# pcodec/pcodec

Measured on AMD Instinct MI355X. Metric: encode+decode GB/s (uncompressed) per chunk, u64/f64 2^18-elem, higher is better.
Workload: dtype u64

## Files before the change

### pcodec_amd/csrc/decode_fast.hip

```cpp
#include "decode_kernel.hip"
#include "pco_cursor.h"
#include "pco_index.h"

namespace pcogfx {

constexpr uint32_t kGrpWinOff = 0;
constexpr uint32_t kGrpVarOff = 448;
constexpr uint32_t kGrpTblOff = 640;
template <uint32_t KQ> struct WalkCfg {
  static constexpr uint32_t kGrpBytes = KQ == 8 ? 4912u : 9904u;
  static constexpr uint32_t kGrpTblBytes = kGrpBytes - kGrpTblOff;
  static constexpr uint32_t kWalkTmpOff = KQ * kGrpBytes;
  static constexpr uint32_t kWalkTmpObOff = kWalkTmpOff + 1056;
  static constexpr uint32_t kWalkLdsBytes = kWalkTmpObOff + 256;
  static constexpr uint32_t kRetryStatus = KQ == 8 ? 101u : 100u;
  static_assert(kGrpBytes % 16 == 0, "chunk slices must stay 16-byte aligned");
  static_assert(kWalkLdsBytes < 65536, "walk entries hold 16-bit LDS addresses");
};
template <uint32_t KQ> __device__ __forceinline__ uint8_t PCO_LDS* walk_lds() { return lds_base() + uni((uint32_t)(threadIdx.x >> 6)) * WalkCfg<KQ>::kWalkLdsBytes; }
__device__ __forceinline__ uint32_t walk_block_id() { return blockIdx.x * (blockDim.x >> 6) + uni((uint32_t)(threadIdx.x >> 6)); }
constexpr uint32_t kTrailDead = 0xffffffffu;
constexpr uint32_t kTrailDoneWord = 8;
constexpr uint32_t kTrailProgressStride = 32;
constexpr bool kTrailDefer = true;
constexpr uint32_t kTrailMaxBins = 64;
constexpr uint32_t kFastMaxBins = 256;
constexpr uint32_t kStatusRetryLegacy = 100;
constexpr uint32_t kStatusRetryK4 = 101;
constexpr uint32_t kStatusNeedHist = 102;
constexpr uint32_t kStatusEmptyRange = 103;

struct DecPlan {
  uint32_t status, n;
  uint32_t mode_kind, mode_k;
  uint64_t mode_base;
  uint32_t num_kind, dtype;
  uint32_t present[3], n_bins[3], max_ob[3], delta_kind[3], delta_order[3], nlps[3];
  uint32_t window_n_log, state_n_log;
  uint64_t moments[2][8];
  uint64_t consumed;
  uint32_t fused, more;
};
struct ReadRef { const uint64_t* from; uint64_t* to; };
struct ReadRec {
  uint32_t route;
  uint32_t b0;
  uint32_t resumed, pad;
  uint64_t mom[2][8];
  uint64_t end_row, end_bit;
  uint32_t end_states[3][4];
};
struct ResumeArgs { const ReadRef* refs; ReadRec* recs; uint32_t walk_cap; };
struct IndexRef { uint64_t* cursors; uint32_t every_batches, k; };
struct IndexArgs { const IndexRef* refs; };
constexpr uint64_t kBinsAreaPerVar = kFastMaxBins * 8 + kFastMaxBins;
constexpr uint64_t kBinsAreaPerTask = 3 * kBinsAreaPerVar;

__device__ __forceinline__ uint32_t make_wentry(uint32_t next_base, uint32_t sym, uint32_t btr, uint32_t ob) { return btr | (ob << 6) | (sym << 13) | (next_base << 21); }

template <class LV, uint32_t KQ>
__device__ __forceinline__ bool fast_build_var_impl(uint32_t q, uint32_t vi, MetaReader& mr, uint8_t PCO_GLOBAL* bins_out, uint32_t& status) {
  constexpr uint32_t kGrpBytes = WalkCfg<KQ>::kGrpBytes, kWalkTmpOff = WalkCfg<KQ>::kWalkTmpOff;
  const uint32_t lane = lane_id();
  uint8_t PCO_LDS* grp = walk_lds<KQ>() + q * kGrpBytes;
  VarInfo PCO_LDS* vinfo = (VarInfo PCO_LDS*)(grp + kGrpVarOff) + vi;
  const uint32_t asl = uni(vinfo->ans_size_log), n_bins = uni(vinfo->n_bins), latent_bits = uni(vinfo->latent_bits);
  const uint32_t T = 1u << asl;
  const uint32_t tbl_addr = (uint32_t)(uintptr_t)walk_lds<KQ>() + q * kGrpBytes + kGrpTblOff + uni(vinfo->off_nodes);
  uint32_t PCO_LDS* entries = (uint32_t PCO_LDS*)(grp + kGrpTblOff + uni(vinfo->off_nodes));
  uint8_t PCO_LDS* obs = walk_lds<KQ>() + WalkCfg<KQ>::kWalkTmpObOff;
  uint8_t PCO_LDS* ob0 = grp + kGrpTblOff + uni(vinfo->off_ob);
  uint32_t PCO_LDS* cum = (uint32_t PCO_LDS*)(walk_lds<KQ>() + kWalkTmpOff);
  uint64_t PCO_GLOBAL* g_low = (uint64_t PCO_GLOBAL*)(bins_out + (uint64_t)vi * kBinsAreaPerVar);
  uint8_t PCO_GLOBAL* g_ob = bins_out + (uint64_t)vi * kBinsAreaPerVar + kFastMaxBins * 8;
  const uint32_t obb = offset_bits_bits(latent_bits);
  const uint32_t bin_bits = asl + latent_bits + obb;
  const uint64_t bins_start = mr.bit;
  uint32_t bad = 0, max_ob = 0, carry = 0;
  for (uint32_t b0 = 0; b0 < n_bins; b0 += 64) {
    const uint32_t b = b0 + lane;
    uint32_t w = 0;
    if (b < n_bins) {
      const uint64_t at = bins_start + (uint64_t)b * bin_bits;
      w = (uint32_t)mr.peek(at, asl) + 1;
      const uint64_t lower = mr.peek(at + asl, latent_bits);
      const uint32_t ob = (uint32_t)mr.peek(at + asl + latent_bits, obb);
      if (ob > latent_bits) bad = 1;
      g_low[b] = lower; g_ob[b] = (uint8_t)ob; obs[b] = (uint8_t)ob;
      if (b == 0) ob0[0] = (uint8_t)ob;
      max_ob = max_ob > ob ? max_ob : ob;
    }
    const uint32_t incl = wave_incl_scan(w);
    if (b < n_bins) cum[b] = carry + incl - w;
    carry += wave_last(incl);
  }
  if (lane == 0) cum[n_bins] = carry;
  mr.bit = bins_start + (uint64_t)n_bins * bin_bits;
  max_ob = uni(wave_max_u32(max_ob));
  if (lane == 0) vinfo->max_ob = max_ob;
  if (!mr.in_bounds()) { status = PCO_GFX_INSUFFICIENT_DATA; return false; }
  if (uni(wave_or_u32(bad))) { status = PCO_GFX_CORRUPTION; return false; }
  if (n_bins == 0) { if (lane == 0) entries[0] = make_wentry(0, 0, 0, 0); wave_sync_lds(); return true; }
  if (carry != T) { status = PCO_GFX_CORRUPTION; return false; }
  wave_sync_lds();
  uint32_t stride = (3 * T) / 5; if ((stride & 1) == 0) stride += 1;
  for (uint32_t t = lane; t < T; t += 64) {
    uint32_t lo = 0, hi = n_bins;
    while (hi - lo > 1) { const uint32_t mid = (lo + hi) >> 1; if (cum[mid] <= t) lo = mid; else hi = mid; }
    entries[(stride * t) & (T - 1)] = lo;
  }
  wave_sync_lds();
// ... 195 lines not shown
  }
  if (!mr.drain_empty_byte()) { if (mr.in_bounds()) { fail(PCO_GFX_CORRUPTION); return; } }
  if (!mr.in_bounds()) { fail(PCO_GFX_INSUFFICIENT_DATA); return; }
  const uint32_t n_in_body = n > nlps[1] ? n - nlps[1] : 0;
  if (n_in_body > 0) for (int vi = 0; vi < 3; vi++) if (present[vi] && uni(vinfo[vi].n_bins) == 0) { fail(PCO_GFX_CORRUPTION); return; }
  out.mode_kind = mode_kind;
  if (lane == 0) {
    plan->status = PCO_GFX_OK; plan->n = n; plan->mode_kind = mode_kind; plan->mode_k = mode_k; plan->mode_base = (uint64_t)mode_base;
    plan->num_kind = num_kind; plan->dtype = dtype; plan->window_n_log = wlog; plan->state_n_log = slog; plan->consumed = 0; plan->fused = 0; plan->more = 0;
    for (int vi = 0; vi < 3; vi++) {
      plan->present[vi] = present[vi]; plan->n_bins[vi] = vinfo[vi].n_bins; plan->max_ob[vi] = vinfo[vi].max_ob;
      plan->delta_kind[vi] = vinfo[vi].delta_kind; plan->delta_order[vi] = vinfo[vi].delta_order; plan->nlps[vi] = nlps[vi];
    }
  }
  out.n = n; out.bitpos = mr.bit;
}

template <class L, uint32_t KQ>
__device__ __noinline__ void fast_front(const PcoGfxDecodeTask& task, uint32_t q, DecPlan PCO_GLOBAL* plan, uint8_t PCO_GLOBAL* bins_out, FrontOut& out, gcptr_u8 meta_p, uint64_t meta_len) { fast_front_impl<L, KQ, false>(task, q, plan, bins_out, out, meta_p, meta_len); }
template <class L, uint32_t KQ>
__device__ __noinline__ void fast_front_range(const PcoGfxDecodeTask& task, uint32_t q, DecPlan PCO_GLOBAL* plan, uint8_t PCO_GLOBAL* bins_out, FrontOut& out, gcptr_u8 meta_p, uint64_t meta_len) { fast_front_impl<L, KQ, false, true>(task, q, plan, bins_out, out, meta_p, meta_len); }

struct ResumeIn { uint64_t row, bitpos; uint32_t states[3][4]; uint32_t resumed; };
template <uint32_t KQ>
__device__ __noinline__ uint32_t resume_front(const uint64_t* from, uint32_t q, uint64_t page_n, uint32_t dtype, uint64_t page_len, uint64_t first, uint64_t count,
                                              uint64_t body_first_bit, uint32_t walk_cap, ReadRec* rec_g, ResumeIn& in) {
  const uint32_t lane = lane_id();
  ReadRec PCO_GLOBAL* rec = (ReadRec PCO_GLOBAL*)rec_g;
  const VarInfo PCO_LDS* vinfo = (const VarInfo PCO_LDS*)(walk_lds<KQ>() + q * WalkCfg<KQ>::kGrpBytes + kGrpVarOff);
  in.row = 0; in.bitpos = body_first_bit;
  uint32_t status = PCO_GFX_OK, resumed = 0;
  if (from != nullptr) {
    const uint64_t PCO_GLOBAL* cw = (const uint64_t PCO_GLOBAL*)from;
    uint64_t w[kCursorMomentWord];
#pragma unroll
    for (uint32_t i = 0; i < kCursorMomentWord; i++) w[i] = uni(cw[i]);
    uint32_t asl[3];
#pragma unroll
    for (int v = 0; v < 3; v++) asl[v] = uni(vinfo[v].present) ? uni(vinfo[v].ans_size_log) : 0u;
    status = cursor_verdict(w, kCursorFull, page_n, dtype, first, body_first_bit, page_len * 8, asl);
    if (status == PCO_GFX_OK) {
      resumed = 1; in.row = w[1]; in.bitpos = w[2];
#pragma unroll
      for (uint32_t v = 0; v < 3; v++) for (uint32_t j = 0; j < 4; j++) in.states[v][j] = cursor_state(w, v, j);
      if (lane < 16) rec->mom[lane >> 3][lane & 7] = cw[kCursorMomentWord + lane];
    }
  }
  if (status == PCO_GFX_OK && range_end_batch(first, count) - (in.row >> 8) > walk_cap) status = PCO_GFX_INVALID_ARGUMENT;
  in.resumed = status == PCO_GFX_OK ? resumed : 0u;
  if (lane == 0) { rec->route = status == PCO_GFX_OK ? 1u : 0u; rec->b0 = (uint32_t)(in.row >> 8); rec->resumed = resumed; rec->pad = 0; }
  return status;
}

struct WalkRegs {
  uint32_t saddr;
  uint32_t e;
  uint32_t bitaddr;
  uint32_t d0, d1, d2;
  uint32_t obsum, symacc;
};

__device__ __forceinline__ void walk_window(WalkRegs& r, uint32_t tot) {
  r.bitaddr += tot;
  const uint32_t PCO_LDS* w = (const uint32_t PCO_LDS*)(uintptr_t)((r.bitaddr >> 3) & ~3u);
  r.d0 = w[0]; r.d1 = w[1]; r.d2 = w[2];
}

template <bool kAgent>
__device__ __forceinline__ void store_syms(uint8_t PCO_GLOBAL* p, uint32_t __attribute__((ext_vector_type(4))) acc) {
  typedef uint32_t u32x4 __attribute__((ext_vector_type(4)));
  if constexpr (kAgent) {
    __asm__ volatile("global_store_dwordx4 %0, %1, off sc1" : : "v"(p), "v"(acc) : "memory");
  } else *(u32x4 PCO_GLOBAL*)p = acc;
}

struct QuadMasks { uint32_t m1, m2, m3, c63; };

template <int K, bool kTail>
__device__ __forceinline__ void walk_step(WalkRegs& r, const QuadMasks& m, uint32_t tbl_addr, bool chain_on) {
  uint32_t e = r.e;
  if (kTail) e = chain_on ? e : 0u;
  const uint32_t p = ((uint32_t)__builtin_amdgcn_update_dpp(0, (int)e, 0x111, 0xf, 0xf, true) & m.m1) +
                     ((uint32_t)__builtin_amdgcn_update_dpp(0, (int)e, 0x112, 0xf, 0xf, true) & m.m2) +
                     ((uint32_t)__builtin_amdgcn_update_dpp(0, (int)e, 0x113, 0xf, 0xf, true) & m.m3);
  const uint32_t x0 = __builtin_amdgcn_alignbit(r.d1, r.d0, r.bitaddr), x1 = __builtin_amdgcn_alignbit(r.d2, r.d1, r.bitaddr);
  const uint64_t xs = (((uint64_t)x1 << 32) | x0) >> (p & 63u);
  const uint32_t v = __builtin_amdgcn_ubfe((uint32_t)xs, 0u, e);
  const uint32_t next = tbl_addr + (((e >> 21) + v) << 2);
  if (kTail) r.saddr = chain_on ? next : r.saddr; else r.saddr = next;
  r.e = *(const uint32_t PCO_LDS*)(uintptr_t)r.saddr;
  __builtin_amdgcn_sched_barrier(0);
  const uint32_t t = p + e;
  walk_window(r, (uint32_t)__builtin_amdgcn_update_dpp(0, (int)t, 0xFF, 0xf, 0xf, true) & m.c63);
  if (K == 0) r.symacc = __builtin_amdgcn_ubfe(e, 13u, 8u); else r.symacc |= __builtin_amdgcn_ubfe(e, 13u, 8u) << (8 * K);
  r.obsum += __builtin_amdgcn_ubfe(e, 6u, 7u);
  __builtin_amdgcn_sched_barrier(0);
}

__device__ __forceinline__ uint32_t block_trail_kinds(const PcoGfxDecodeTask* tasks, const uint32_t* task_ids, uint32_t n_ids, uint32_t wb, const MetaRef* metas) {
  const uint32_t lane = lane_id(), bi = wb * 8 + (lane & 7u);
  bool one = false, two = false;
  if (lane < 8 && bi < n_ids) {
    const uint32_t ti = task_ids ? task_ids[bi] : bi;
    const PcoGfxDecodeTask t = tasks[ti];
    const bool wrapped = (t.flags & PCO_GFX_TASK_WRAPPED_PAGE) != 0;
    const uint32_t fmt = wrapped ? (t.flags >> 8) & 0xffu : ((t.flags & PCO_GFX_TASK_ONE_CHUNK) && ((t.flags >> 8) & 0xffu) ? (t.flags >> 8) & 0xffu : 4u);
    gcptr_u8 mp = (gcptr_u8)t.src + 4; uint64_t mlen = t.src_len >= 4 ? t.src_len - 4 : 0;
    if (wrapped) { if (metas != nullptr && metas[ti].p != nullptr) { mp = (gcptr_u8)metas[ti].p; mlen = metas[ti].len; } else { mp = (gcptr_u8)t.src; mlen = t.src_len; } }
    if ((t.flags & (PCO_GFX_TASK_META_ONLY | PCO_GFX_TASK_HAS_FILE_HEADER)) == 0 && mlen >= 20 && fmt >= 3 && fmt <= 4) {
      const uint64_t w = load_u64_le(mp);
      const uint32_t mode = (uint32_t)w & 15u;
      if (mode == kClassic) {
        const uint32_t dv = (uint32_t)(w >> 4) & 15u;
        const uint32_t n_bins = (uint32_t)(w >> (dv == kDeltaConsecutive ? 16 : 12)) & 0x7fffu;
        one = (dv == kDeltaNone || dv == kDeltaConsecutive) && n_bins > 1 && n_bins <= kTrailMaxBins;
      } else if (mode == kIntMult || mode == kFloatMult || mode == kFloatQuant) {
        const uint32_t at = 4u + (mode == kFloatQuant ? kBitsQuantK : (uint32_t)dtype_bits(t.dtype));
        const uint64_t w2 = load_u64_le(mp + (at >> 3));
        const uint32_t dv = (uint32_t)(w2 >> (at & 7u)) & 15u;
        two = dv == kDeltaNone || dv == kDeltaConsecutive;
      }
    }
  }
  return (uni((uint32_t)__any(one)) ? 1u : 0u) | (uni((uint32_t)__any(two)) ? 2u : 0u);
}
__device__ __forceinline__ bool block_has_trail_candidate(const PcoGfxDecodeTask* tasks, const uint32_t* task_ids, uint32_t n_ids, uint32_t wb, const MetaRef* metas) {
  return block_trail_kinds(tasks, task_ids, n_ids, wb, metas) != 0;
}

template <class L, uint32_t kWQ, bool kTrail, bool kRange = false, bool kResume = false, bool kIndex = false>
__device__ __forceinline__ void dec_walk_body(const PcoGfxDecodeTask* tasks, const uint32_t* task_ids, uint32_t n_ids, DecPlan* plans,
                                              uint8_t* bins_area, uint8_t* sym_area, uint64_t sym_stride, uint64_t* offpos_area, uint64_t offpos_stride,
                                              uint32_t accept_status, PcoGfxTaskResult* results, uint32_t* progress, const MetaRef* metas,
                                              const RangeRef* ranges = nullptr, ResumeArgs rz = ResumeArgs{nullptr, nullptr, 0}, IndexArgs ix = IndexArgs{nullptr}) {
  static_assert(!kTrail || !kRange, "range tasks never take the publishing walker");
  static_assert(!kResume || kRange, "a resumed walk is a range walk");
  static_assert(!kIndex || (kRange && !kResume), "an index walk is a range walk from the page's start");
  static_assert(!kTrail || kWQ == 8, "the trailing expanders follow the eight-chunk walker");
  const uint32_t wb = walk_block_id();
  if ((uint64_t)wb * kWQ >= n_ids) return;
  constexpr uint32_t kGrpBytes = WalkCfg<kWQ>::kGrpBytes;
  if constexpr (kTrail) __builtin_amdgcn_s_setprio(3);
  const uint32_t lane = lane_id();
  const uint32_t slot = lane >> 2, j = lane & 3;
  if constexpr (kTrail) {
    if (!block_has_trail_candidate(tasks, task_ids, n_ids, wb, metas)) {
      if (lane < 8) __hip_atomic_store(progress + (uint64_t)wb * kTrailProgressStride + lane, kTrailDead, __ATOMIC_RELAXED, __HIP_MEMORY_SCOPE_AGENT);
// ... 49 lines not shown
        }
      } else if (lane == 0) (rz.recs + ti)->route = 0;
    }
    wave_sync_lds();
  }
  const uint32_t slice = (slot < kWQ ? slot : 0u) * kGrpBytes;
  uint8_t PCO_LDS* gbase = walk_lds<kWQ>() + slice;
  const uint32_t lds0 = (uint32_t)(uintptr_t)walk_lds<kWQ>();
  uint64_t PCO_LDS* win = (uint64_t PCO_LDS*)(gbase + kGrpWinOff);
  VarInfo PCO_LDS* vinfo = (VarInfo PCO_LDS*)(gbase + kGrpVarOff);
  uint32_t n_rem = my_n, batch = 0, cur_v = 0, status = PCO_GFX_OK, present_mask = 0, nlps1 = 0;
  if (my_active) {
    present_mask = (vinfo[0].present ? 1u : 0u) | 2u | (vinfo[2].present ? 4u : 0u);
    nlps1 = vinfo[1].delta_kind == kDeltaConsecutive ? vinfo[1].delta_order : (vinfo[1].delta_kind == kDeltaLookback ? (1u << vinfo[1].state_n_log) : 0u);
    cur_v = (present_mask & 1u) ? 0u : 1u;
    if constexpr (kResume) { batch = my_b0; n_rem = my_n - my_b0 * kBatchN; }
    if (n_rem == 0) my_active = 0;
    st0 = lds0 + slice + kGrpTblOff + vinfo[0].off_nodes + 4u * st0;
    st1 = lds0 + slice + kGrpTblOff + vinfo[1].off_nodes + 4u * st1;
    st2 = lds0 + slice + kGrpTblOff + vinfo[2].off_nodes + 4u * st2;
  }
  bool my_fused = false;
  uint32_t my_fused_kind = 0;
  uint32_t PCO_GLOBAL* my_progress = nullptr;
  if constexpr (kTrail) {
    if (my_active && slot < kWQ) {
      const bool prim_ok = vinfo[0].present == 0 && vinfo[1].n_bins >= 1 && vinfo[1].n_bins <= kTrailMaxBins && vinfo[1].max_ob <= 16 &&
                           (vinfo[1].delta_kind == kDeltaConsecutive ? vinfo[1].delta_order <= 2 : vinfo[1].delta_kind == kDeltaNone);
      if (vinfo[2].present == 0) { if (prim_ok && my_mode == kClassic && vinfo[1].n_bins > 1) my_fused_kind = 1; }
      else if (prim_ok && (my_mode == kIntMult || my_mode == kFloatMult || my_mode == kFloatQuant) && vinfo[2].n_bins >= 1 && vinfo[2].n_bins <= kTrailMaxBins &&
               vinfo[2].max_ob <= 16 && vinfo[2].delta_kind == kDeltaNone && (vinfo[1].n_bins > 1 || vinfo[2].n_bins > 1)) my_fused_kind = 2;
      my_fused = my_fused_kind != 0;
    }
    if (slot < kWQ) my_progress = (uint32_t PCO_GLOBAL*)progress + (uint64_t)wb * kTrailProgressStride + slot;
    if (j == 0 && my_fused) ((DecPlan PCO_GLOBAL*)plans + my_ti)->fused = my_fused_kind;
    __builtin_amdgcn_fence(__ATOMIC_RELEASE, "agent");
    if (j == 0 && slot < kWQ) __hip_atomic_store((uint32_t*)my_progress, my_fused ? 1u : kTrailDead, __ATOMIC_RELAXED, __HIP_MEMORY_SCOPE_AGENT);
  }

  typedef uint32_t u32x4 __attribute__((ext_vector_type(4)));
  QuadMasks qm = {j >= 1 ? ~0u : 0u, j >= 2 ? ~0u : 0u, j >= 3 ? ~0u : 0u, 63u};
  asm volatile("" : "+v"(qm.m1), "+v"(qm.m2), "+v"(qm.m3), "+v"(qm.c63));
  u32x4 d_acc[4] = {{0u, 0u, 0u, 0u}, {0u, 0u, 0u, 0u}, {0u, 0u, 0u, 0u}, {0u, 0u, 0u, 0u}};
  uint32_t d_ngrp = 0, issued_batches = 0; uint8_t PCO_GLOBAL* d_sym_out = nullptr;
  uint64_t d_off_val = 0; uint64_t* d_off_ptr = nullptr;
  auto flush_deferred = [&]() {
#pragma unroll
    for (int g = 0; g < 4; g++) if ((uint32_t)g < d_ngrp) store_syms<true>(d_sym_out + 64 * g, d_acc[g]);
    d_ngrp = 0;
    if (d_off_ptr) __hip_atomic_store(d_off_ptr, d_off_val, __ATOMIC_RELAXED, __HIP_MEMORY_SCOPE_AGENT);
    d_off_ptr = nullptr;
  };
  uint64_t touch_prev = my_bitpos >> 3; uint32_t touch_r0 = 0, touch_r1 = 0;
  while (__any(my_active != 0)) {
    uint32_t cnt = 0, nb = 0, asl = 0, off_ob = 0, off_nodes = 0;
    bool walk = false;
    if (my_active) {
      const VarInfo PCO_LDS* vi = vinfo + cur_v;
      nb = vi->n_bins; asl = vi->ans_size_log; off_ob = vi->off_ob; off_nodes = vi->off_nodes;
      const uint32_t batch_n = n_rem < kBatchN ? n_rem : kBatchN;
      if (cur_v == 0) { const uint32_t lim = n_rem > nlps1 ? n_rem - nlps1 : 0; cnt = lim < batch_n ? lim : batch_n; }
      else {
        const uint32_t nl = cur_v == 1 ? nlps1 : (vi->delta_kind == kDeltaConsecutive ? vi->delta_order : (vi->delta_kind == kDeltaLookback ? (1u << vi->state_n_log) : 0u));
        const uint32_t rem = n_rem > nl ? n_rem - nl : 0; cnt = rem < kBatchN ? rem : kBatchN;
      }
      walk = cnt > 0 && nb > 1;
    }
    const uint64_t q0 = my_bitpos >> 6;
    WalkRegs r;
    r.saddr = cur_v == 0 ? st0 : (cur_v == 1 ? st1 : st2);
    const uint32_t win_addr = lds0 + slice + kGrpWinOff, rel0 = (uint32_t)(my_bitpos & 63);
    r.bitaddr = 8u * win_addr + rel0; r.obsum = 0; r.symacc = 0; r.e = 0; r.d0 = r.d1 = r.d2 = 0;
    if (walk) {
      const uint32_t nq = ((((rel0 + cnt * asl + 63u) >> 6) + 3u) + 1u) & ~1u;
      uint64_t lo[7], hi[7];
      if ((q0 + nq) * 8 <= my_len + 16) {
#pragma unroll
        for (int k = 0; k < 7; k++) {
          const uint32_t qi = 2 * j + 8 * k, qc = qi < nq ? qi : nq - 2;
          lo[k] = load_u64_le(my_src + (q0 + qc) * 8); hi[k] = load_u64_le(my_src + (q0 + qc) * 8 + 8);
        }
      } else {
#pragma unroll
        for (int k = 0; k < 7; k++) {
          const uint32_t qi = 2 * j + 8 * k;
          lo[k] = 0; hi[k] = 0;
          if (qi < nq) { lo[k] = load_u64_le_safe(my_src, (q0 + qi) * 8, my_len + 16); hi[k] = load_u64_le_safe(my_src, (q0 + qi + 1) * 8, my_len + 16); }
        }
      }
#pragma unroll
      for (int k = 0; k < 7; k++) { const uint32_t qi = 2 * j + 8 * k; if (qi < nq) { win[qi] = lo[k]; win[qi + 1] = hi[k]; } }
    }
    wave_sync_lds();
    if constexpr (kTrail) {
      __asm__ volatile("s_waitcnt vmcnt(0)" ::: "memory");
      if (my_fused && j == 0 && status == PCO_GFX_OK) __hip_atomic_store((uint32_t*)my_progress, 1u + issued_batches, __ATOMIC_RELAXED, __HIP_MEMORY_SCOPE_AGENT);
      if constexpr (kTrailDefer) { flush_deferred(); issued_batches = batch; }
      else issued_batches = batch;
    }
    ((uint32_t PCO_LDS*)(walk_lds<kWQ>() + WalkCfg<kWQ>::kWalkTmpOff))[lane] = touch_r0 ^ touch_r1;
    if (walk) {
      const uint64_t cur = q0 * 8, pred = cur + (cur - touch_prev);
      touch_prev = cur;
      const uint64_t line0 = (pred & ~(uint64_t)127) - (pred >= 128 ? 128u : 0u);
      const uint64_t a0 = line0 + 128u * j, a1 = a0 + 512u;
      touch_r0 = load_u32_le(my_src + (a0 + 4 <= my_len ? a0 : 0));
      touch_r1 = load_u32_le(my_src + (a1 + 4 <= my_len ? a1 : 0));
    }
    const uint32_t obs_addr = lds0 + slice + kGrpTblOff + off_ob, tbl_addr = lds0 + slice + kGrpTblOff + off_nodes;
    uint8_t PCO_GLOBAL* sym_out = (uint8_t PCO_GLOBAL*)sym_area + ((uint64_t)(my_ti == 0xffffffffu ? 0u : my_ti) * 3 + cur_v) * sym_stride + (uint64_t)(kResume ? batch - my_b0 : batch) * kBatchN + 16 * j;
    if (walk) {
      r.e = *(const uint32_t PCO_LDS*)(uintptr_t)r.saddr;
      walk_window(r, 0u);
      constexpr bool defer = kTrail && kTrailDefer;
      if constexpr (defer) d_sym_out = sym_out;
      if (__all(!walk || cnt == kBatchN)) {
#pragma unroll
        for (uint32_t grp = 0; grp < 4; grp++) {
          u32x4 acc;
#pragma unroll
          for (int b = 0; b < 4; b++) {
            walk_step<0, false>(r, qm, tbl_addr, true);
            walk_step<1, false>(r, qm, tbl_addr, true);
            walk_step<2, false>(r, qm, tbl_addr, true);
            walk_step<3, false>(r, qm, tbl_addr, true);
            acc[b] = r.symacc;
          }
          if constexpr (defer) d_acc[grp] = acc; else store_syms<kTrail>(sym_out + 64 * grp, acc);
        }
        if constexpr (defer) d_ngrp = 4;
      } else {
        const uint32_t steps = (cnt + 3) >> 2;
        if constexpr (defer) d_ngrp = (steps + 15) >> 4;
#pragma unroll
        for (uint32_t grp = 0; grp < 4; grp++) {
          if (grp * 16 >= steps) break;
          u32x4 acc = {0u, 0u, 0u, 0u};
#pragma unroll
          for (int b = 0; b < 4; b++) {
            const uint32_t g = grp * 16 + b * 4;
            if (g < steps) {
              r.symacc = 0;
              if (g + 0 < steps) walk_step<0, true>(r, qm, tbl_addr, 4 * (g + 0) + j < cnt);
              if (g + 1 < steps) walk_step<1, true>(r, qm, tbl_addr, 4 * (g + 1) + j < cnt);
              if (g + 2 < steps) walk_step<2, true>(r, qm, tbl_addr, 4 * (g + 2) + j < cnt);
              if (g + 3 < steps) walk_step<3, true>(r, qm, tbl_addr, 4 * (g + 3) + j < cnt);
              acc[b] = r.symacc;
            }
          }
          if constexpr (defer) d_acc[grp] = acc; else store_syms<kTrail>(sym_out + 64 * grp, acc);
        }
      }
      if (cur_v == 0) st0 = r.saddr; else if (cur_v == 1) st1 = r.saddr; else st2 = r.saddr;
    }
    if (my_active) {
      uint32_t obq = r.obsum;
      obq += (uint32_t)__builtin_amdgcn_update_dpp(0, (int)obq, 0xB1, 0xf, 0xf, false);
      obq += (uint32_t)__builtin_amdgcn_update_dpp(0, (int)obq, 0x4E, 0xf, 0xf, false);
      const uint64_t ans_end = walk ? (q0 << 6) + (r.bitaddr - 8u * win_addr) : my_bitpos;
      uint64_t ob_total = 0;
      if (cnt > 0) ob_total = walk ? (uint64_t)obq : (nb == 1 ? (uint64_t)cnt * *(const uint8_t PCO_LDS*)(uintptr_t)obs_addr : 0ull);
      if (cnt > 0 && j == 0) {
        uint64_t* op = offpos_area + ((uint64_t)my_ti * 3 + cur_v) * offpos_stride + (kResume ? batch - my_b0 : batch);
        if constexpr (kTrail && kTrailDefer) { d_off_ptr = op; d_off_val = ans_end; }
        else if constexpr (kTrail) __hip_atomic_store(op, ans_end, __ATOMIC_RELAXED, __HIP_MEMORY_SCOPE_AGENT);
        else *op = ans_end;
      }
      my_bitpos = ans_end + ob_total;
      if (my_bitpos > my_len * 8) { status = PCO_GFX_INSUFFICIENT_DATA; my_active = 0; }
      uint32_t nv = cur_v + 1;
      while (nv < 3 && !((present_mask >> nv) & 1u)) nv++;
      if (nv >= 3) {
        const uint32_t batch_n = n_rem < kBatchN ? n_rem : kBatchN;
        n_rem -= batch_n; batch++;
        if constexpr (kIndex) {
          const uint32_t cs = status == PCO_GFX_OK ? index_slot(batch, my_every, my_k) : kIndexNoSlot;
          if (cs != kIndexNoSlot) {
            uint64_t PCO_GLOBAL* cw = my_cur + (uint64_t)cs * kCursorWords;
            uint32_t PCO_GLOBAL* sw = (uint32_t PCO_GLOBAL*)(cw + kCursorStateWord);
            const uint32_t tb = lds0 + slice + kGrpTblOff;
            sw[j] = (st0 - tb - vinfo[0].off_nodes) >> 2; sw[4 + j] = (st1 - tb - vinfo[1].off_nodes) >> 2; sw[8 + j] = (st2 - tb - vinfo[2].off_nodes) >> 2;
            if (j == 0) { cw[1] = (uint64_t)batch * kBatchN; cw[2] = my_bitpos; }
          }
        }
        nv = (present_mask & 1u) ? 0u : 1u;
        if (n_rem == 0) my_active = 0;
        if constexpr (kRange) { if (batch >= my_bend) my_active = 0; }
      }
      cur_v = nv;
    }
    wave_sync_lds();
  }
  if constexpr (kTrail) {
    flush_deferred();
    __asm__ volatile("s_waitcnt vmcnt(0)" ::: "memory");
    if (my_fused && j == 0) __hip_atomic_store((uint32_t*)my_progress, status == PCO_GFX_OK ? 1u + batch : kTrailDead, __ATOMIC_RELAXED, __HIP_MEMORY_SCOPE_AGENT);
  }
  if (my_ti != 0xffffffffu && j == 0 && slot < kWQ) {
    DecPlan PCO_GLOBAL* plan = (DecPlan PCO_GLOBAL*)plans + my_ti;
    if (my_front_ok) {
      uint64_t bit = my_bitpos;
      bool open_end = false;
      if constexpr (kRange) open_end = status == PCO_GFX_OK && n_rem != 0;
      if (status == PCO_GFX_OK && !open_end) {
        const uint32_t sh = (uint32_t)(bit & 7);
        if (sh) { const uint64_t byte = bit >> 3; const uint32_t b = byte < my_len ? my_src[byte] : 0u; if ((b >> sh) != 0) status = PCO_GFX_CORRUPTION; bit += 8 - sh; }
        if (bit > my_len * 8) status = PCO_GFX_INSUFFICIENT_DATA;
      }
      if (!kIndex && (my_flags & PCO_GFX_TASK_WRAPPED_PAGE) && status != PCO_GFX_OK) status = kStatusRetryLegacy;
      if (status == PCO_GFX_OK) {
        uint64_t byte = bit >> 3;
        if (my_flags & PCO_GFX_TASK_WRAPPED_PAGE) { }
        else if (my_flags & PCO_GFX_TASK_ONE_CHUNK) {
          if (byte < my_len && my_src[byte] != 0) plan->more = 1u;
          else if (byte < my_len) { byte += 1; plan->more = 2u; }
          else if (my_flags & PCO_GFX_TASK_HAS_FILE_HEADER) status = PCO_GFX_INSUFFICIENT_DATA;
        } else if (my_flags & PCO_GFX_TASK_HAS_FILE_HEADER) {
          if (byte >= my_len) status = PCO_GFX_INSUFFICIENT_DATA;
          else if (my_src[byte] != 0) status = kStatusRetryLegacy;
          else byte += 1;
        } else if (byte < my_len) status = kStatusRetryLegacy;
        plan->consumed = open_end ? 0 : byte;
      }
      plan->status = status;
      if constexpr (kResume) { ReadRec PCO_GLOBAL* rec = (ReadRec PCO_GLOBAL*)rz.recs + my_ti; rec->end_row = my_n - n_rem; rec->end_bit = my_bitpos; }
      if constexpr (kTrail) {
        if (my_fused && status != kStatusRetryLegacy) {
          PcoGfxTaskResult r; r.n_out = status == PCO_GFX_OK ? my_n : 0; r.consumed = plan->consumed; r.status = status; r.aux = plan->more;
          results[my_ti] = r;
        }
      }
    }
  }
  if constexpr (kResume) {
    if (my_ti != 0xffffffffu && slot < kWQ && my_front_ok) {
      ReadRec PCO_GLOBAL* rec = (ReadRec PCO_GLOBAL*)rz.recs + my_ti;
      const uint32_t tb = lds0 + slice + kGrpTblOff;
      rec->end_states[0][j] = (st0 - tb - vinfo[0].off_nodes) >> 2; rec->end_states[1][j] = (st1 - tb - vinfo[1].off_nodes) >> 2; rec->end_states[2][j] = (st2 - tb - vinfo[2].off_nodes) >> 2;
    }
  }
}

template <class L, uint32_t kWQ>
__global__ __launch_bounds__(256) void dec_walk_kernel(const PcoGfxDecodeTask* tasks, const uint32_t* task_ids, uint32_t n_ids, DecPlan* plans,
                                                      uint8_t* bins_area, uint8_t* sym_area, uint64_t sym_stride, uint64_t* offpos_area, uint64_t offpos_stride,
// ... 504 lines not shown
```

### pcodec_amd/csrc/pco_gfx.hip

```cpp
#include "pco_host.h"
#include "pco_half.h"

#include <algorithm>
#include <atomic>
#include <chrono>
#include <thread>
#include <mutex>
#include <condition_variable>
#include <functional>
#include <sched.h>
#include <pthread.h>
#include <sys/syscall.h>
#include <unistd.h>
#include <cstdlib>
#include <cstring>
#include <memory>
#include <unordered_map>

#include "pco_auto_host.inc"
#include "decode_kernel.hip"
#include "decode_trail.hip"
#include "encode_kernels.hip"
#include "encode_lookback.hip"
#include "encode_conv1.hip"
// ... 274 lines not shown
  const size_t n_again = flat_ids.size();
  if (!n_again) return;
  std::vector<uint64_t> offs; uint64_t hist_bytes = 0;
  for (uint32_t i : flat_ids) { offs.push_back(hist_bytes); hist_bytes += ((tasks[i].dst_cap * (uint64_t)(dtype_bits(tasks[i].dtype) / 8)) + 255) & ~(uint64_t)255; }
  uint8_t* d_hist = (uint8_t*)c.ws.dec_hist.ensure(hist_bytes + n_again * 12 + 256);
  uint64_t* d_hoff = (uint64_t*)(d_hist + ((hist_bytes + 15) & ~(uint64_t)15));
  uint32_t* d_again = (uint32_t*)(d_hoff + n_again);
  PCO_HIP_CHECK(hipMemcpyAsync(d_hoff, offs.data(), n_again * 8, hipMemcpyHostToDevice, c.stream));
  PCO_HIP_CHECK(hipMemcpyAsync(d_again, flat_ids.data(), n_again * 4, hipMemcpyHostToDevice, c.stream));
  uint8_t* tbl = (uint8_t*)c.ws.tbl_ws.ensure(std::min<size_t>(n_again, kGeneralGrid) * kTblWsBytes);
  for (int g = 0; g < 4; g++) {
    const uint32_t cnt = (uint32_t)(goff[g + 1] - goff[g]);
    if (!cnt) continue;
    launch_width(g, GeneralDecodeStep{c, kDecodeKernelNames[g][kNameGeneral], cnt, d_again + goff[g], tbl, nullptr, 0u, 0u, d_hist, d_hoff + goff[g], (uint32_t)PCO_GFX_UNSUPPORTED});
  }
  PCO_HIP_CHECK(hipGetLastError());
  read_decode_results(c, n_tasks, results);
}

}

using namespace pcogfx;

extern "C" {

int pco_gfx_last_status(void) { return g_err.status; }
const char* pco_gfx_last_error(void) { return g_err.msg.c_str(); }
int pco_gfx_device_count(void) { int n = 0; if (hipGetDeviceCount(&n) != hipSuccess) return 0; return n; }
void pco_gfx_release_workspace(void) {
  try { Workspace& w = workspace(); if (w.has_last && w.last_event) (void)hipEventSynchronize(w.last_event); w.release_all(); } catch (...) {}
}

size_t pco_gfx_workspace_bytes(void) {
  try {
    static const bool trace = std::getenv("PCO_GFX_TRACE") != nullptr;
    if (trace) fprintf(stderr, "[pco_gfx trace] workspace: %s\n", workspace().device_report().c_str());
    return workspace().device_bytes();
  } catch (...) { return 0; }
}

static unsigned long long trail_stat(int which) {
  try {
    Workspace& w = workspace();
    const unsigned long long acc = which == 0 ? w.acc_givebacks : w.acc_marked;
    if (!w.dec_stats.p) return acc;
    if (w.has_last && w.last_event) (void)hipEventSynchronize(w.last_event);
    uint32_t v[2] = {0, 0};
    if (hipMemcpy(v, w.dec_stats.p, 8, hipMemcpyDeviceToHost) != hipSuccess) return acc;
    return acc + v[which];
  } catch (...) { return 0; }
}
unsigned long long pco_gfx_trail_givebacks(void) { return trail_stat(0); }
unsigned long long pco_gfx_trail_marked(void) { return trail_stat(1); }
unsigned long long pco_gfx_strict_histogram_fallbacks(void) {
  try {
    Workspace& w = workspace();
    if (!w.enc_strict.p) return w.acc_strict;
    if (w.has_last && w.last_event) (void)hipEventSynchronize(w.last_event);
    uint32_t v = 0;
    if (hipMemcpy(&v, w.enc_strict.p, 4, hipMemcpyDeviceToHost) != hipSuccess) return w.acc_strict;
    return w.acc_strict + v;
  } catch (...) { return 0; }
}

void pco_gfx_profile_begin(void) {
  for (auto& r : g_prof.recs) { g_prof.give(r.a); g_prof.give(r.b); }
  g_prof.recs.clear(); g_prof.on = true;
}
int pco_gfx_profile_end(char* names, size_t names_cap, float* ms, int cap) {
  g_prof.on = false;
  int n = 0; size_t pos = 0;
  for (auto& r : g_prof.recs) {
    float t = 0.f;
    (void)hipEventSynchronize(r.b);
    (void)hipEventElapsedTime(&t, r.a, r.b);
    if (n < cap) {
      const size_t len = std::strlen(r.name) + 1;
      if (names && pos + len <= names_cap) { std::memcpy(names + pos, r.name, len); pos += len; }
      if (ms) ms[n] = t;
      n++;
    }
    g_prof.give(r.a); g_prof.give(r.b);
  }
  g_prof.recs.clear();
  return n;
}

size_t pco_gfx_guarantee_file_size(size_t n, unsigned char dtype, uint64_t max_page_n) {
  const int bits = dtype_bits(dtype);
  if (!bits) return 0;
  std::vector<size_t> pages;
  n_per_page(max_page_n, n, pages);
  size_t res = guarantee_standalone_header_size() + 1;
  for (size_t p : pages) res += guarantee_standalone_chunk_size(bits, p);
  return res;
}
size_t pco_standalone_guarantee_file_size(size_t n, unsigned char dtype) { return pco_gfx_guarantee_file_size(n, dtype, 0); }
size_t pco_gfx_guarantee_chunk_size(size_t n, unsigned char dtype) {
  const int bits = dtype_bits(dtype);
  return bits ? guarantee_standalone_chunk_size(bits, n) : 0;
}

size_t pco_gfx_write_standalone_header(void* dst, size_t dst_cap, uint64_t n_hint, unsigned char uniform_dtype) {
  HostBitWriter w;
  w.write(0x216f6370u, 32); w.write(3, 8); w.write(uniform_dtype, 8);
  const uint32_t power = n_hint == 0 ? 1 : (64 - (uint32_t)__builtin_clzll(n_hint));
// ... 343 lines not shown
```

Measured before the change: 1770.

## Reorder walk entry fields, shorten step critical path, add steady-state loop

Walk table entries now store next_base in the middle bits and the symbol in the top byte. The next-address base can then be computed before the bit-extract, and symbols are packed with v_perm instead of shift/or. For 8-chunk slices the 64-bit shift is replaced by a single alignbit, which relies on table bits staying at most 10. A steady-state path skips per-batch VarInfo reads and variable iteration when only variable 1 is present with full batches. The staging, publish and touch code is moved into lambdas, and timing instrumentation is added behind a compile-time flag.

```diff
diff --git a/pcodec_amd/csrc/decode_fast.hip b/pcodec_amd/csrc/decode_fast.hip
--- a/pcodec_amd/csrc/decode_fast.hip
+++ b/pcodec_amd/csrc/decode_fast.hip
@@ -56,7 +56,8 @@
 constexpr uint64_t kBinsAreaPerVar = kFastMaxBins * 8 + kFastMaxBins;
 constexpr uint64_t kBinsAreaPerTask = 3 * kBinsAreaPerVar;
 
-__device__ __forceinline__ uint32_t make_wentry(uint32_t next_base, uint32_t sym, uint32_t btr, uint32_t ob) { return btr | (ob << 6) | (sym << 13) | (next_base << 21); }
+constexpr uint32_t kWentryNextShift = 13, kWentryNextBits = 11, kWentrySymShift = 24;
+__device__ __forceinline__ uint32_t make_wentry(uint32_t next_base, uint32_t sym, uint32_t btr, uint32_t ob) { return btr | (ob << 6) | (next_base << kWentryNextShift) | (sym << kWentrySymShift); }
 
 template <class LV, uint32_t KQ>
 __device__ __forceinline__ bool fast_build_var_impl(uint32_t q, uint32_t vi, MetaReader& mr, uint8_t PCO_GLOBAL* bins_out, uint32_t& status) {
@@ -358,6 +359,18 @@
   return status;
 }
 
+#ifdef PCO_WALK_TIMING
+static __device__ unsigned long long pco_walk_timing[8];
+#define PCO_WT_DECL uint64_t wt_sum[5] = {0, 0, 0, 0, 0}, wt_prev = __builtin_amdgcn_s_memtime(); uint32_t wt_rounds = 0
+#define PCO_WT(i) do { if constexpr (kTrail) { __builtin_amdgcn_sched_barrier(0); const uint64_t wt_now = __builtin_amdgcn_s_memtime(); __asm__ volatile("s_waitcnt lgkmcnt(0)" ::: "memory"); \
+    wt_sum[i] += wt_now - wt_prev; wt_prev = wt_now; if (i == 0) wt_rounds++; __builtin_amdgcn_sched_barrier(0); } } while (0)
+#define PCO_WT_DONE do { if constexpr (kTrail) { if (wb == 0 && lane == 0) { for (int i = 0; i < 5; i++) pco_walk_timing[i] = wt_sum[i]; pco_walk_timing[5] = wt_rounds; } } } while (0)
+#else
+#define PCO_WT_DECL do { } while (0)
+#define PCO_WT(i) do { } while (0)
+#define PCO_WT_DONE do { } while (0)
+#endif
+
 struct WalkRegs {
   uint32_t saddr;
   uint32_t e;
@@ -382,23 +395,32 @@
 
 struct QuadMasks { uint32_t m1, m2, m3, c63; };
 
-template <int K, bool kTail>
+template <int K, bool kTail, uint32_t KQ>
 __device__ __forceinline__ void walk_step(WalkRegs& r, const QuadMasks& m, uint32_t tbl_addr, bool chain_on) {
+  static_assert(KQ != 8 || WalkCfg<8>::kGrpTblBytes < (4u << 11), "the one-instruction shift by p needs bits_to_read <= 10: no ans_size_log 11 table in an 8-chunk slice");
   uint32_t e = r.e;
   if (kTail) e = chain_on ? e : 0u;
   const uint32_t p = ((uint32_t)__builtin_amdgcn_update_dpp(0, (int)e, 0x111, 0xf, 0xf, true) & m.m1) +
                      ((uint32_t)__builtin_amdgcn_update_dpp(0, (int)e, 0x112, 0xf, 0xf, true) & m.m2) +
                      ((uint32_t)__builtin_amdgcn_update_dpp(0, (int)e, 0x113, 0xf, 0xf, true) & m.m3);
+  uint32_t nb = __builtin_amdgcn_ubfe(e, kWentryNextShift, kWentryNextBits);
+  asm("" : "+v"(nb));
+  uint32_t pre = tbl_addr + (nb << 2);
+  asm("" : "+v"(pre));
+  __builtin_amdgcn_sched_barrier(0);
   const uint32_t x0 = __builtin_amdgcn_alignbit(r.d1, r.d0, r.bitaddr), x1 = __builtin_amdgcn_alignbit(r.d2, r.d1, r.bitaddr);
-  const uint64_t xs = (((uint64_t)x1 << 32) | x0) >> (p & 63u);
-  const uint32_t v = __builtin_amdgcn_ubfe((uint32_t)xs, 0u, e);
-  const uint32_t next = tbl_addr + (((e >> 21) + v) << 2);
+  uint32_t xs;
+  if constexpr (KQ == 8) xs = __builtin_amdgcn_alignbit(x1, x0, p);
+  else xs = (uint32_t)((((uint64_t)x1 << 32) | x0) >> (p & 63u));
+  const uint32_t v = __builtin_amdgcn_ubfe(xs, 0u, e);
+  const uint32_t next = pre + (v << 2);
   if (kTail) r.saddr = chain_on ? next : r.saddr; else r.saddr = next;
   r.e = *(const uint32_t PCO_LDS*)(uintptr_t)r.saddr;
   __builtin_amdgcn_sched_barrier(0);
   const uint32_t t = p + e;
   walk_window(r, (uint32_t)__builtin_amdgcn_update_dpp(0, (int)t, 0xFF, 0xf, 0xf, true) & m.c63);
-  if (K == 0) r.symacc = __builtin_amdgcn_ubfe(e, 13u, 8u); else r.symacc |= __builtin_amdgcn_ubfe(e, 13u, 8u) << (8 * K);
+  if (K == 0) r.symacc = e >> kWentrySymShift;
+  else r.symacc = __builtin_amdgcn_perm(e, r.symacc, K == 1 ? 0x03020700u : (K == 2 ? 0x03070100u : 0x07020100u));
   r.obsum += __builtin_amdgcn_ubfe(e, 6u, 7u);
   __builtin_amdgcn_sched_barrier(0);
 }
@@ -554,52 +576,36 @@
     d_off_ptr = nullptr;
   };
   uint64_t touch_prev = my_bitpos >> 3; uint32_t touch_r0 = 0, touch_r1 = 0;
-  while (__any(my_active != 0)) {
-    uint32_t cnt = 0, nb = 0, asl = 0, off_ob = 0, off_nodes = 0;
-    bool walk = false;
-    if (my_active) {
-      const VarInfo PCO_LDS* vi = vinfo + cur_v;
-      nb = vi->n_bins; asl = vi->ans_size_log; off_ob = vi->off_ob; off_nodes = vi->off_nodes;
-      const uint32_t batch_n = n_rem < kBatchN ? n_rem : kBatchN;
-      if (cur_v == 0) { const uint32_t lim = n_rem > nlps1 ? n_rem - nlps1 : 0; cnt = lim < batch_n ? lim : batch_n; }
-      else {
-        const uint32_t nl = cur_v == 1 ? nlps1 : (vi->delta_kind == kDeltaConsecutive ? vi->delta_order : (vi->delta_kind == kDeltaLookback ? (1u << vi->state_n_log) : 0u));
-        const uint32_t rem = n_rem > nl ? n_rem - nl : 0; cnt = rem < kBatchN ? rem : kBatchN;
-      }
-      walk = cnt > 0 && nb > 1;
-    }
-    const uint64_t q0 = my_bitpos >> 6;
-    WalkRegs r;
-    r.saddr = cur_v == 0 ? st0 : (cur_v == 1 ? st1 : st2);
-    const uint32_t win_addr = lds0 + slice + kGrpWinOff, rel0 = (uint32_t)(my_bitpos & 63);
-    r.bitaddr = 8u * win_addr + rel0; r.obsum = 0; r.symacc = 0; r.e = 0; r.d0 = r.d1 = r.d2 = 0;
-    if (walk) {
-      const uint32_t nq = ((((rel0 + cnt * asl + 63u) >> 6) + 3u) + 1u) & ~1u;
-      uint64_t lo[7], hi[7];
-      if ((q0 + nq) * 8 <= my_len + 16) {
-#pragma unroll
-        for (int k = 0; k < 7; k++) {
-          const uint32_t qi = 2 * j + 8 * k, qc = qi < nq ? qi : nq - 2;
-          lo[k] = load_u64_le(my_src + (q0 + qc) * 8); hi[k] = load_u64_le(my_src + (q0 + qc) * 8 + 8);
-        }
-      } else {
-#pragma unroll
-        for (int k = 0; k < 7; k++) {
-          const uint32_t qi = 2 * j + 8 * k;
-          lo[k] = 0; hi[k] = 0;
-          if (qi < nq) { lo[k] = load_u64_le_safe(my_src, (q0 + qi) * 8, my_len + 16); hi[k] = load_u64_le_safe(my_src, (q0 + qi + 1) * 8, my_len + 16); }
-        }
-      }
-#pragma unroll
-      for (int k = 0; k < 7; k++) { const uint32_t qi = 2 * j + 8 * k; if (qi < nq) { win[qi] = lo[k]; win[qi + 1] = hi[k]; } }
-    }
-    wave_sync_lds();
+  PCO_WT_DECL;
+  auto stage = [&](uint64_t q0, uint32_t nq) {
+    uint64_t lo[7], hi[7];
+    if ((q0 + nq) * 8 <= my_len + 16) {
+#pragma unroll
+      for (int k = 0; k < 7; k++) {
+        const uint32_t qi = 2 * j + 8 * k, qc = qi < nq ? qi : nq - 2;
+        lo[k] = load_u64_le(my_src + (q0 + qc) * 8); hi[k] = load_u64_le(my_src + (q0 + qc) * 8 + 8);
+      }
+    } else {
+#pragma unroll
+      for (int k = 0; k < 7; k++) {
+        const uint32_t qi = 2 * j + 8 * k;
+        lo[k] = 0; hi[k] = 0;
+        if (qi < nq) { lo[k] = load_u64_le_safe(my_src, (q0 + qi) * 8, my_len + 16); hi[k] = load_u64_le_safe(my_src, (q0 + qi + 1) * 8, my_len + 16); }
+      }
+    }
+    PCO_WT(1);
+#pragma unroll
+    for (int k = 0; k < 7; k++) { const uint32_t qi = 2 * j + 8 * k; if (qi < nq) { win[qi] = lo[k]; win[qi + 1] = hi[k]; } }
+  };
+  auto publish = [&]() {
     if constexpr (kTrail) {
       __asm__ volatile("s_waitcnt vmcnt(0)" ::: "memory");
       if (my_fused && j == 0 && status == PCO_GFX_OK) __hip_atomic_store((uint32_t*)my_progress, 1u + issued_batches, __ATOMIC_RELAXED, __HIP_MEMORY_SCOPE_AGENT);
       if constexpr (kTrailDefer) { flush_deferred(); issued_batches = batch; }
       else issued_batches = batch;
     }
+  };
+  auto touch = [&](bool walk, uint64_t q0) {
     ((uint32_t PCO_LDS*)(walk_lds<kWQ>() + WalkCfg<kWQ>::kWalkTmpOff))[lane] = touch_r0 ^ touch_r1;
     if (walk) {
       const uint64_t cur = q0 * 8, pred = cur + (cur - touch_prev);
@@ -609,6 +615,64 @@
       touch_r0 = load_u32_le(my_src + (a0 + 4 <= my_len ? a0 : 0));
       touch_r1 = load_u32_le(my_src + (a1 + 4 <= my_len ? a1 : 0));
     }
+  };
+  auto full_steps = [&](WalkRegs& r, uint32_t tbl_addr, uint8_t PCO_GLOBAL* sym_out) {
+    constexpr bool defer = kTrail && kTrailDefer;
+    PCO_WT(3);
+#pragma unroll
+    for (uint32_t grp = 0; grp < 4; grp++) {
+      u32x4 acc;
+#pragma unroll
+      for (int b = 0; b < 4; b++) {
+        walk_step<0, false, kWQ>(r, qm, tbl_addr, true);
+        walk_step<1, false, kWQ>(r, qm, tbl_addr, true);
+        walk_step<2, false, kWQ>(r, qm, tbl_addr, true);
+        walk_step<3, false, kWQ>(r, qm, tbl_addr, true);
+        acc[b] = r.symacc;
+      }
+      if constexpr (defer) d_acc[grp] = acc; else store_syms<kTrail>(sym_out + 64 * grp, acc);
+    }
+    if constexpr (defer) d_ngrp = 4;
+    PCO_WT(4);
+  };
+  bool steady = false;
+  uint32_t h_var = 0;
+  if constexpr (!kRange) {
+    const bool fits = !my_active || (present_mask == 2u && vinfo[1].n_bins > 1);
+    steady = __all(fits);
+#if defined(PCO_WALK_TIMING) && PCO_WALK_TIMING == 2
+    steady = false;
+#endif
+    if (steady && my_active) h_var = vinfo[1].ans_size_log | (vinfo[1].off_nodes << 16);
+  }
+  while (__any(my_active != 0)) {
+    uint32_t cnt = 0, nb = 0, asl = 0, off_ob = 0, off_nodes = 0;
+    bool walk = false;
+    if constexpr (!kRange) { if (steady) steady = __all(!my_active || n_rem >= kBatchN + nlps1); }
+    if (steady) {
+      if (my_active) { cnt = kBatchN; nb = 2; asl = h_var & 0xffffu; off_nodes = h_var >> 16; walk = true; }
+    } else if (my_active) {
+      const VarInfo PCO_LDS* vi = vinfo + cur_v;
+      nb = vi->n_bins; asl = vi->ans_size_log; off_ob = vi->off_ob; off_nodes = vi->off_nodes;
+      const uint32_t batch_n = n_rem < kBatchN ? n_rem : kBatchN;
+      if (cur_v == 0) { const uint32_t lim = n_rem > nlps1 ? n_rem - nlps1 : 0; cnt = lim < batch_n ? lim : batch_n; }
+      else {
+        const uint32_t nl = cur_v == 1 ? nlps1 : (vi->delta_kind == kDeltaConsecutive ? vi->delta_order : (vi->delta_kind == kDeltaLookback ? (1u << vi->state_n_log) : 0u));
+        const uint32_t rem = n_rem > nl ? n_rem - nl : 0; cnt = rem < kBatchN ? rem : kBatchN;
+      }
+      walk = cnt > 0 && nb > 1;
+    }
+    const uint64_t q0 = my_bitpos >> 6;
+    WalkRegs r;
+    r.saddr = cur_v == 0 ? st0 : (cur_v == 1 ? st1 : st2);
+    const uint32_t win_addr = lds0 + slice + kGrpWinOff, rel0 = (uint32_t)(my_bitpos & 63);
+    r.bitaddr = 8u * win_addr + rel0; r.obsum = 0; r.symacc = 0; r.e = 0; r.d0 = r.d1 = r.d2 = 0;
+    PCO_WT(0);
+    if (walk) stage(q0, ((((rel0 + cnt * asl + 63u) >> 6) + 3u) + 1u) & ~1u);
+    wave_sync_lds();
+    publish();
+    PCO_WT(2);
+    touch(walk, q0);
     const uint32_t obs_addr = lds0 + slice + kGrpTblOff + off_ob, tbl_addr = lds0 + slice + kGrpTblOff + off_nodes;
     uint8_t PCO_GLOBAL* sym_out = (uint8_t PCO_GLOBAL*)sym_area + ((uint64_t)(my_ti == 0xffffffffu ? 0u : my_ti) * 3 + cur_v) * sym_stride + (uint64_t)(kResume ? batch - my_b0 : batch) * kBatchN + 16 * j;
     if (walk) {
@@ -616,22 +680,8 @@
       walk_window(r, 0u);
       constexpr bool defer = kTrail && kTrailDefer;
       if constexpr (defer) d_sym_out = sym_out;
-      if (__all(!walk || cnt == kBatchN)) {
-#pragma unroll
-        for (uint32_t grp = 0; grp < 4; grp++) {
-          u32x4 acc;
-#pragma unroll
-          for (int b = 0; b < 4; b++) {
-            walk_step<0, false>(r, qm, tbl_addr, true);
-            walk_step<1, false>(r, qm, tbl_addr, true);
-            walk_step<2, false>(r, qm, tbl_addr, true);
-            walk_step<3, false>(r, qm, tbl_addr, true);
-            acc[b] = r.symacc;
-          }
-          if constexpr (defer) d_acc[grp] = acc; else store_syms<kTrail>(sym_out + 64 * grp, acc);
-        }
-        if constexpr (defer) d_ngrp = 4;
-      } else {
+      if (__all(!walk || cnt == kBatchN)) full_steps(r, tbl_addr, sym_out);
+      else {
         const uint32_t steps = (cnt + 3) >> 2;
         if constexpr (defer) d_ngrp = (steps + 15) >> 4;
 #pragma unroll
@@ -643,10 +693,10 @@
             const uint32_t g = grp * 16 + b * 4;
             if (g < steps) {
               r.symacc = 0;
-              if (g + 0 < steps) walk_step<0, true>(r, qm, tbl_addr, 4 * (g + 0) + j < cnt);
-              if (g + 1 < steps) walk_step<1, true>(r, qm, tbl_addr, 4 * (g + 1) + j < cnt);
-              if (g + 2 < steps) walk_step<2, true>(r, qm, tbl_addr, 4 * (g + 2) + j < cnt);
-              if (g + 3 < steps) walk_step<3, true>(r, qm, tbl_addr, 4 * (g + 3) + j < cnt);
+              if (g + 0 < steps) walk_step<0, true, kWQ>(r, qm, tbl_addr, 4 * (g + 0) + j < cnt);
+              if (g + 1 < steps) walk_step<1, true, kWQ>(r, qm, tbl_addr, 4 * (g + 1) + j < cnt);
+              if (g + 2 < steps) walk_step<2, true, kWQ>(r, qm, tbl_addr, 4 * (g + 2) + j < cnt);
+              if (g + 3 < steps) walk_step<3, true, kWQ>(r, qm, tbl_addr, 4 * (g + 3) + j < cnt);
               acc[b] = r.symacc;
             }
           }
@@ -671,8 +721,9 @@
       my_bitpos = ans_end + ob_total;
       if (my_bitpos > my_len * 8) { status = PCO_GFX_INSUFFICIENT_DATA; my_active = 0; }
       uint32_t nv = cur_v + 1;
-      while (nv < 3 && !((present_mask >> nv) & 1u)) nv++;
-      if (nv >= 3) {
+      if (steady) { n_rem -= kBatchN; batch++; nv = 1; if (n_rem == 0) my_active = 0; }
+      else while (nv < 3 && !((present_mask >> nv) & 1u)) nv++;
+      if (!steady && nv >= 3) {
         const uint32_t batch_n = n_rem < kBatchN ? n_rem : kBatchN;
         n_rem -= batch_n; batch++;
         if constexpr (kIndex) {
@@ -693,6 +744,7 @@
     }
     wave_sync_lds();
   }
+  PCO_WT_DONE;
   if constexpr (kTrail) {
     flush_deferred();
     __asm__ volatile("s_waitcnt vmcnt(0)" ::: "memory");
diff --git a/pcodec_amd/csrc/pco_gfx.hip b/pcodec_amd/csrc/pco_gfx.hip
--- a/pcodec_amd/csrc/pco_gfx.hip
+++ b/pcodec_amd/csrc/pco_gfx.hip
@@ -350,6 +350,12 @@
 }
 unsigned long long pco_gfx_trail_givebacks(void) { return trail_stat(0); }
 unsigned long long pco_gfx_trail_marked(void) { return trail_stat(1); }
+#ifdef PCO_WALK_TIMING
+int pco_gfx_walk_timing(unsigned long long* out) {
+  if (hipDeviceSynchronize() != hipSuccess) return PCO_GFX_DEVICE_ERROR;
+  return hipMemcpyFromSymbol(out, HIP_SYMBOL(pcogfx::pco_walk_timing), 8 * sizeof(unsigned long long)) == hipSuccess ? PCO_GFX_OK : PCO_GFX_DEVICE_ERROR;
+}
+#endif
 unsigned long long pco_gfx_strict_histogram_fallbacks(void) {
   try {
     Workspace& w = workspace();
```

After: 1774 (median of 3 runs). About the same (+0.2%).
